# zju3dv/Diffuman4D

Measured on NVIDIA H100. Metric: unet_window_denoise_steps_per_sec, higher is better.
Workload: dtype bf16

## Files before the change

diffuman4d_b200/csrc/common.cuh:

```cuda
#pragma once
#include <cuda.h>
#include <cuda_bf16.h>
#include <cuda_runtime.h>
#include <stdint.h>
#include <string>

namespace d4d {

typedef __nv_bfloat16 bf16;

void set_error(const std::string& msg);
#define D4D_CUDA_OK(expr)                                                                        \
  do {                                                                                           \
    cudaError_t _e = (expr);                                                                     \
    if (_e != cudaSuccess) {                                                                     \
      d4d::set_error(std::string(#expr) + " failed: " + cudaGetErrorString(_e) + " @" + __FILE__ + \
                     ":" + std::to_string(__LINE__));                                            \
      return 2;                                                                                  \
    }                                                                                            \
  } while (0)
#define D4D_REQUIRE(cond, msg)                                                                   \
  do {                                                                                           \
    if (!(cond)) {                                                                               \
      d4d::set_error(std::string("invalid argument: ") + msg + " (" #cond ") @" + __FILE__ + ":" + \
                     std::to_string(__LINE__));                                                  \
      return 1;                                                                                  \
    }                                                                                            \
  } while (0)

int make_tmap_2d(CUtensorMap* out, const void* base, uint64_t rows, uint64_t cols, uint64_t ld,
                 uint32_t box_cols, uint32_t box_rows, int swizzle_bytes);
int make_tmap_nhwc_store(CUtensorMap* out, void* base, uint64_t n, uint64_t h, uint64_t w, uint64_t c, uint32_t box_w,
                         uint32_t box_h, uint32_t box_n);
int make_tmap_nhwc(CUtensorMap* out, const void* base, uint64_t n, uint64_t h, uint64_t w, uint64_t c,
                   uint32_t box_c, uint32_t box_w, uint32_t box_h, uint32_t box_n, int swizzle_bytes, int stride = 1);

#ifdef __CUDACC__
__device__ __forceinline__ uint32_t smem_u32(const void* p) {
  return static_cast<uint32_t>(__cvta_generic_to_shared(p));
}
__device__ __forceinline__ bool elect_one() {
  uint32_t pred = 0;
  asm volatile(
      "{\n\t.reg .b32 rx;\n\t.reg .pred px;\n\t"
      "elect.sync rx|px, 0xffffffff;\n\t"
      "selp.b32 %0, 1, 0, px;\n\t}\n"
      : "=r"(pred));
  return pred != 0;
// ... 28 lines not shown
#endif
__device__ __forceinline__ void mbar_wait(uint64_t* bar, uint32_t parity) {
  uint32_t spins = 0;
  while (!mbar_try_wait(bar, parity)) {
    if (++spins > D4D_SPIN_LIMIT) {
      printf("d4d: mbarrier timeout block=(%d,%d) thread=%d bar=%u parity=%u\n", blockIdx.x, blockIdx.y,
             threadIdx.x, smem_u32(bar), parity);
      __trap();
    }
  }
}

__device__ __forceinline__ void fence_proxy_async_smem() {
  asm volatile("fence.proxy.async.shared::cta;" ::: "memory");
}
__device__ __forceinline__ void pdl_wait() { asm volatile("griddepcontrol.wait;" ::: "memory"); }
__device__ __forceinline__ void pdl_launch_dependents() { asm volatile("griddepcontrol.launch_dependents;" ::: "memory"); }
template <int R> __device__ __forceinline__ void setmaxnreg_dec() { asm volatile("setmaxnreg.dec.sync.aligned.u32 %0;" ::"n"(R)); }
template <int R> __device__ __forceinline__ void setmaxnreg_inc() { asm volatile("setmaxnreg.inc.sync.aligned.u32 %0;" ::"n"(R)); }

__device__ __forceinline__ void tma_prefetch_desc(const CUtensorMap* t) {
  asm volatile("prefetch.tensormap [%0];" ::"l"(reinterpret_cast<uint64_t>(t)) : "memory");
}
__device__ __forceinline__ void tma_load_2d(void* dst, const CUtensorMap* t, uint64_t* bar, int c0, int c1) {
  asm volatile(
      "cp.async.bulk.tensor.2d.shared::cluster.global.tile.mbarrier::complete_tx::bytes [%0], [%1, {%3, %4}], [%2];"
      ::"r"(smem_u32(dst)), "l"(reinterpret_cast<uint64_t>(t)), "r"(smem_u32(bar)), "r"(c0), "r"(c1)
      : "memory");
}
__device__ __forceinline__ void tma_load_4d(void* dst, const CUtensorMap* t, uint64_t* bar, int c0, int c1, int c2,
                                            int c3) {
  asm volatile(
      "cp.async.bulk.tensor.4d.shared::cluster.global.tile.mbarrier::complete_tx::bytes [%0], [%1, {%3, %4, %5, %6}], [%2];"
      ::"r"(smem_u32(dst)), "l"(reinterpret_cast<uint64_t>(t)), "r"(smem_u32(bar)), "r"(c0), "r"(c1), "r"(c2),
      "r"(c3)
      : "memory");
}

__device__ __forceinline__ void tma_store_2d(const CUtensorMap* t, const void* src, int c0, int c1) {
  asm volatile("cp.async.bulk.tensor.2d.global.shared::cta.bulk_group [%0, {%2, %3}], [%1];"
               ::"l"(reinterpret_cast<uint64_t>(t)), "r"(smem_u32(src)), "r"(c0), "r"(c1) : "memory");
}
__device__ __forceinline__ void tma_store_4d(const CUtensorMap* t, const void* src, int c0, int c1, int c2, int c3) {
  asm volatile("cp.async.bulk.tensor.4d.global.shared::cta.bulk_group [%0, {%2, %3, %4, %5}], [%1];"
               ::"l"(reinterpret_cast<uint64_t>(t)), "r"(smem_u32(src)), "r"(c0), "r"(c1), "r"(c2), "r"(c3) : "memory");
}
__device__ __forceinline__ void bulk_commit_group() { asm volatile("cp.async.bulk.commit_group;" ::: "memory"); }
template <int N> __device__ __forceinline__ void bulk_wait_group_read() {
  asm volatile("cp.async.bulk.wait_group.read %0;" ::"n"(N) : "memory");
}
template <int N> __device__ __forceinline__ void bulk_wait_group() {
  asm volatile("cp.async.bulk.wait_group %0;" ::"n"(N) : "memory");
}

__device__ __forceinline__ uint32_t pack_bf16x2(float lo, float hi) {
  __nv_bfloat162 v = __floats2bfloat162_rn(lo, hi);
  return *reinterpret_cast<uint32_t*>(&v);
}
__device__ __forceinline__ float2 unpack_bf16x2(uint32_t u) {
  __nv_bfloat162 v = *reinterpret_cast<__nv_bfloat162*>(&u);
// ... 17 lines not shown
```

diffuman4d_b200/csrc/gemm_wgmma.cu:

```cuda
#include "kernels.h"
#include "wgmma.cuh"

namespace d4d {

namespace {

constexpr int BLOCK_M = 128;
constexpr int BLOCK_K = 64;
constexpr int A_BYTES = BLOCK_M * BLOCK_K * 2;
constexpr int BAR_BYTES = 1024;
constexpr int NUM_THREADS = 384;
constexpr int MAX_SMEM = 227 * 1024;

template <int BN>
struct GemmCfg {
  static constexpr int STAGE_BYTES = A_BYTES + BN * BLOCK_K * 2;
  static constexpr int STAGES_FIT = (MAX_SMEM - 1024 - BAR_BYTES) / STAGE_BYTES;
  static constexpr int STAGES = STAGES_FIT > 8 ? 8 : STAGES_FIT;
  static constexpr int SMEM = 1024 + BAR_BYTES + STAGES * STAGE_BYTES;
};

struct TileCoord {
  int m0;
  int n_img0, y0, x0;
  int pa, pb;
};

template <bool kConv>
__device__ __forceinline__ void tile_coords(const GemmKernelArgs& a, int m_tile, TileCoord& t) {
  if (!kConv) {
    t.m0 = m_tile * BLOCK_M;
    t.n_img0 = t.y0 = t.x0 = 0;
    t.pa = t.pb = 0;
  } else {
// ... 20 lines not shown
    valid = row < a.M;
    img = a.rows_per_image > 0 ? static_cast<int>(row / a.rows_per_image) : 0;
  } else {
    const int bx = rr % a.BW;
    const int r2 = rr / a.BW;
    const int by = r2 % a.BH;
    const int bn = r2 / a.BH;
    const int x = tc.x0 + bx, y = tc.y0 + by, n = tc.n_img0 + bn;
    valid = (x < a.W) && (y < a.H) && (n < a.n_img);
    row = (static_cast<long long>(n) * a.out_H + (y * a.out_sy + a.out_oy + tc.pa)) * a.out_W + (x * a.out_sx + a.out_ox + tc.pb);
    img = n;
  }
}

enum : int { E_BIAS = 1, E_ROWVEC = 2, E_ACT = 4, E_RES = 8, E_STATS = 16, E_KV = 32, E_ALL = 63 };

template <int BN, bool kGeglu, bool kConv, int kEpi>
__global__ void __launch_bounds__(NUM_THREADS, 1)
gemm_wgmma_kernel(const __grid_constant__ CUtensorMap tmap_a, const __grid_constant__ CUtensorMap tmap_a2,
                  const __grid_constant__ CUtensorMap tmap_b, const GemmKernelArgs a) {
  using Cfg = GemmCfg<BN>;
  constexpr int STAGES = Cfg::STAGES;
  extern __shared__ uint8_t smem_raw[];
  uint8_t* smem = reinterpret_cast<uint8_t*>((reinterpret_cast<uintptr_t>(smem_raw) + 1023) & ~uintptr_t(1023));
  uint64_t* full = reinterpret_cast<uint64_t*>(smem);
  uint64_t* empty = full + STAGES;
  uint8_t* ring = smem + BAR_BYTES;

  const int warp = __shfl_sync(0xffffffffu, threadIdx.x >> 5, 0);
  const int lane = threadIdx.x & 31;
  const int total_tiles = a.m_tiles * a.n_tiles;

  if (threadIdx.x == 0) {
    tma_prefetch_desc(&tmap_a);
    tma_prefetch_desc(&tmap_b);
    if (a.kb_split < a.k_blocks) tma_prefetch_desc(&tmap_a2);
    for (int i = 0; i < STAGES; ++i) {
      mbar_init(&full[i], 1);
      mbar_init(&empty[i], 2);
    }
    fence_mbar_init();
  }
  __syncthreads();
  pdl_wait();
  pdl_launch_dependents();

  if (warp < 4) {
    setmaxnreg_dec<40>();
    if (threadIdx.x == 0) {
      const uint32_t tx_bytes = A_BYTES + static_cast<uint32_t>(a.block_n) * BLOCK_K * 2;
      int stage = 0;
      uint32_t phase = 0;
      for (int tile = blockIdx.x; tile < total_tiles; tile += gridDim.x) {
        const int m_tile = tile / a.n_tiles;
        const int n_tile = tile % a.n_tiles;
// ... 18 lines not shown
          }
          if (++stage == STAGES) { stage = 0; phase ^= 1; }
        }
      }
    }
    return;
  }

  setmaxnreg_inc<232>();
  const int wg = (warp >> 2) - 1;
  const int wq = warp & 3;
  const bool wg_leader = (threadIdx.x & 127) == 0;
  const int r_base = wg * 64 + wq * 16 + (lane >> 2);
  const int c_base = 2 * (lane & 3);
  const uint32_t ring_u32 = smem_u32(ring);

  int stage = 0;
  uint32_t phase = 0;
  float acc[BN / 2];
  for (int tile = blockIdx.x; tile < total_tiles; tile += gridDim.x) {
    const int m_tile = tile / a.n_tiles;
    const int n_tile = tile % a.n_tiles;
    TileCoord tc;
    tile_coords<kConv>(a, m_tile, tc);
    const int n0 = n_tile * a.block_n;

    int prev_stage = -1;
    for (int kb = 0; kb < a.k_blocks; ++kb) {
      mbar_wait(&full[stage], phase);
      const uint32_t sa = ring_u32 + stage * Cfg::STAGE_BYTES + wg * 64 * 128;
      const uint32_t sb = ring_u32 + stage * Cfg::STAGE_BYTES + A_BYTES;
      const uint64_t adesc = make_wgmma_desc(sa, 16, 1024);
      const uint64_t bdesc = make_wgmma_desc(sb, 16, 1024);
      wgmma_fence();
#pragma unroll
      for (int k = 0; k < BLOCK_K / 16; ++k) {
        const int scale_d = (kb | k) != 0 ? 1 : 0;
        if constexpr (BN == 64) wgmma_ss_n64(acc, adesc + 2 * k, bdesc + 2 * k, scale_d);
        else if constexpr (BN == 128) wgmma_ss_n128(acc, adesc + 2 * k, bdesc + 2 * k, scale_d);
        else wgmma_ss_n256(acc, adesc + 2 * k, bdesc + 2 * k, scale_d);
      }
      wgmma_commit();
      wgmma_wait<1>();
      if (prev_stage >= 0 && wg_leader) mbar_arrive(&empty[prev_stage]);
      prev_stage = stage;
      if (++stage == STAGES) { stage = 0; phase ^= 1; }
    }
    wgmma_wait<0>();
    wgmma_fence_regs(acc);
    if (wg_leader) mbar_arrive(&empty[prev_stage]);

    long long rows[2];
    int imgs[2];
    bool valid[2];
    row_of<kConv>(a, tc, r_base, rows[0], imgs[0], valid[0]);
    row_of<kConv>(a, tc, r_base + 8, rows[1], imgs[1], valid[1]);

    if constexpr (kGeglu) {
      const bool has_bias = (kEpi & E_BIAS) && a.bias != nullptr;
#pragma unroll
      for (int p = 0; p < BN / 16; ++p) {
        if (16 * p >= a.block_n || n0 + 16 * p >= a.N) break;
        float2 ba = make_float2(0.f, 0.f), bg = make_float2(0.f, 0.f);
        if (has_bias) {
          ba = __ldg(reinterpret_cast<const float2*>(a.bias + n0 + 16 * p + c_base));
          bg = __ldg(reinterpret_cast<const float2*>(a.bias + n0 + 16 * p + 8 + c_base));
        }
        const int ocol = n0 / 2 + 8 * p + c_base;
#pragma unroll
        for (int h = 0; h < 2; ++h) {
          if (!valid[h]) continue;
          const float a0 = acc[8 * p + 2 * h] + ba.x, a1 = acc[8 * p + 2 * h + 1] + ba.y;
          const float g0 = acc[8 * p + 4 + 2 * h] + bg.x, g1 = acc[8 * p + 4 + 2 * h + 1] + bg.y;
          *reinterpret_cast<uint32_t*>(a.out + static_cast<size_t>(rows[h]) * a.ldo + ocol) =
              pack_bf16x2(a0 * gelu_erf_f(g0), a1 * gelu_erf_f(g1));
        }
      }
    } else {
      const bool has_bias = (kEpi & E_BIAS) && a.bias != nullptr, has_rv = (kEpi & E_ROWVEC) && a.rowvec != nullptr;
      const bool has_res = (kEpi & E_RES) && a.residual != nullptr, has_stats = (kEpi & E_STATS) && a.stats != nullptr;
      const bool has_act = (kEpi & E_ACT) && a.act == 1, has_scale = (kEpi & E_ACT) && a.out_scale != 1.0f;
      const bool has_kv = (kEpi & E_KV) && a.kv_world > 0;
      const long long row0 = __shfl_sync(0xffffffffu, rows[0], 0);
      const bool stats_on = has_stats && __shfl_sync(0xffffffffu, valid[0] ? 1 : 0, 0);
      const int stats_img = !kConv ? static_cast<int>(row0 / a.stats_rows) : __shfl_sync(0xffffffffu, imgs[0], 0);
#pragma unroll
      for (int j = 0; j < BN / 8; ++j) {
        const int cl = 8 * j + c_base;
        const int col = n0 + cl;
        if (8 * j >= a.block_n || n0 + 8 * j >= a.N) break;
        float2 b2 = make_float2(0.f, 0.f);
        if (has_bias) b2 = __ldg(reinterpret_cast<const float2*>(a.bias + col));
        float sv[2][2];
#pragma unroll
        for (int h = 0; h < 2; ++h) {
          sv[h][0] = sv[h][1] = 0.f;
          if (!valid[h]) continue;
          float f0 = acc[4 * j + 2 * h] + b2.x, f1 = acc[4 * j + 2 * h + 1] + b2.y;
          if (has_rv) {
            const float2 v = unpack_bf16x2(*reinterpret_cast<const uint32_t*>(a.rowvec + static_cast<size_t>(imgs[h]) * a.ld_rowvec + col));
            f0 += v.x; f1 += v.y;
          }
          if (has_act) { f0 = silu_f(f0); f1 = silu_f(f1); }
          if (has_scale) { f0 *= a.out_scale; f1 *= a.out_scale; }
          if (has_res) {
            const float2 v = unpack_bf16x2(*reinterpret_cast<const uint32_t*>(a.residual + static_cast<size_t>(rows[h]) * a.ld_res + col));
            f0 += v.x; f1 += v.y;
          }
          const uint32_t o = pack_bf16x2(f0, f1);
          if (has_stats) {
            const float2 rv = unpack_bf16x2(o);
            sv[h][0] = rv.x; sv[h][1] = rv.y;
          }
          if (has_kv && col >= a.kv_col0) {
            const long long half = rows[h] / a.kv_rows_local;
            const long long grow = half * a.kv_rows_global + a.kv_row_offset + (rows[h] - half * a.kv_rows_local);
            const size_t off = static_cast<size_t>(grow) * a.kv_ld + (col - a.kv_col0);
#pragma unroll 1
            for (int rk = 0; rk < a.kv_world; ++rk) *reinterpret_cast<uint32_t*>(a.kv_dst[rk] + off) = o;
          } else {
            *reinterpret_cast<uint32_t*>(a.out + static_cast<size_t>(rows[h]) * a.ldo + col) = o;
          }
        }
        if (has_stats) {
          float s0 = sv[0][0] + sv[1][0], s1 = sv[0][1] + sv[1][1];
          float q0 = sv[0][0] * sv[0][0] + sv[1][0] * sv[1][0], q1 = sv[0][1] * sv[0][1] + sv[1][1] * sv[1][1];
#pragma unroll
          for (int m = 4; m < 32; m <<= 1) {
            s0 += __shfl_xor_sync(0xffffffffu, s0, m);
            s1 += __shfl_xor_sync(0xffffffffu, s1, m);
            q0 += __shfl_xor_sync(0xffffffffu, q0, m);
            q1 += __shfl_xor_sync(0xffffffffu, q1, m);
          }
          if (stats_on && lane < 4) {
            unsigned long long* st = reinterpret_cast<unsigned long long*>(a.stats) + (static_cast<size_t>(stats_img) * a.N + col) * 2;
            atomicAdd(st + 0, static_cast<unsigned long long>(__float2ll_rn(s0 * kGnSumScale)));
            atomicAdd(st + 1, static_cast<unsigned long long>(__float2ll_rn(q0 * kGnSqScale)));
            atomicAdd(st + 2, static_cast<unsigned long long>(__float2ll_rn(s1 * kGnSumScale)));
            atomicAdd(st + 3, static_cast<unsigned long long>(__float2ll_rn(q1 * kGnSqScale)));
          }
        }
      }
    }
  }
}

}

int gemm_prepare(const GemmDesc& d, GemmLaunch* L) {
  D4D_REQUIRE(d.N % 16 == 0, "GEMM N must be a multiple of 16");
  D4D_REQUIRE(d.out != nullptr && d.A != nullptr && d.Wt != nullptr, "null operand");
  GemmKernelArgs& a = L->args;
  memset(&a, 0, sizeof(a));
  int dev = 0, sms = 0;
  D4D_CUDA_OK(cudaGetDevice(&dev));
  D4D_CUDA_OK(cudaDeviceGetAttribute(&sms, cudaDevAttrMultiProcessorCount, dev));
  int bn = d.block_n;
  if (bn <= 0) {
    const long long rows = d.conv ? static_cast<long long>(d.n_img) * d.H * d.W : d.M;
    const long long m_tiles_est = (rows + BLOCK_M - 1) / BLOCK_M;
    long long best_cost = -1;
    for (int c = 64; c <= 256; c *= 2) {
      const long long tiles = m_tiles_est * ((d.N + c - 1) / c);
      const long long waves = (tiles + sms - 1) / sms;
      const long long cost = waves * (c + 64) + (static_cast<long long>((d.N + c - 1) / c) * c - d.N) / 4;
      if (best_cost < 0 || cost <= best_cost) { best_cost = cost; bn = c; }
    }
  }
  D4D_REQUIRE(bn >= 16 && bn <= 256 && bn % 16 == 0 && (d.block_n <= 0 || d.N % bn == 0), "no valid block_n");
  a.block_n = bn;
  a.n_tiles = (d.N + bn - 1) / bn;
  a.N = d.N;
  a.bias = d.bias;
  a.rowvec = d.rowvec;
  a.ld_rowvec = d.ld_rowvec;
  a.rows_per_image = d.rows_per_image;
  a.residual = d.residual;
// ... 24 lines not shown
    D4D_REQUIRE(d.A2 == nullptr || d.K1 % BLOCK_K == 0, "two-source GEMM needs K1 % 64 == 0");
    a.mode = 0;
    a.M = d.M;
    a.m_tiles = (d.M + BLOCK_M - 1) / BLOCK_M;
    a.kb_split = (d.K1 + BLOCK_K - 1) / BLOCK_K;
    const int kb2 = d.A2 ? (d.K2 + BLOCK_K - 1) / BLOCK_K : 0;
    a.k_blocks = a.kb_split + kb2;
    const int K = d.K1 + (d.A2 ? d.K2 : 0);
    if (int rc = make_tmap_2d(&L->tmap_a, d.A, d.M, d.K1, d.lda, BLOCK_K, BLOCK_M, 128)) return rc;
    if (d.A2) {
      if (int rc = make_tmap_2d(&L->tmap_a2, d.A2, d.M, d.K2, d.lda2, BLOCK_K, BLOCK_M, 128)) return rc;
    } else {
      L->tmap_a2 = L->tmap_a;
    }
    if (int rc = make_tmap_2d(&L->tmap_b, d.Wt, d.N, K, K, BLOCK_K, bn, 128)) return rc;
  } else {
    D4D_REQUIRE(d.Cin % 8 == 0, "conv Cin must be a multiple of 8");
    D4D_REQUIRE(d.conv_kind >= 0 && d.conv_kind <= 3, "conv_kind");
    D4D_REQUIRE(d.conv_kind != 1 || (d.H % 2 == 0 && d.W % 2 == 0), "stride-2 conv needs even H, W");
    a.mode = 1;
    a.n_img = d.n_img; a.Cin = d.Cin;
    a.in_stride = 1; a.out_sy = a.out_sx = 1; a.out_oy = a.out_ox = 0;
    a.n_phases = 1;
    if (d.conv_kind >= 2) {
      const int pa = d.conv_kind == 3 ? 0 : d.up_a, pb = d.conv_kind == 3 ? 0 : d.up_b;
      a.n_taps = 4;
      for (int t = 0; t < 4; ++t) {
        a.tap_dy[t] = static_cast<signed char>((t >> 1) + pa - 1);
        a.tap_dx[t] = static_cast<signed char>((t & 1) + pb - 1);
      }
// ... 15 lines not shown
    a.k_blocks = a.n_taps * a.cin_blocks;
    a.kb_split = a.k_blocks;
    int bw = 16; while (bw > a.W) bw >>= 1;
    int bh = 128 / bw; while (bh > a.H && bh > 1) bh >>= 1;
    int bnimg = 128 / (bw * bh);
    D4D_REQUIRE(bw * bh * bnimg == 128 && bnimg <= 256, "conv tile shape");
    D4D_REQUIRE(d.stats == nullptr || (bw * bh) % 32 == 0, "statistics need 32-row warps inside one image");
    a.BW = bw; a.BH = bh; a.BN = bnimg;
    a.tiles_x = (a.W + bw - 1) / bw;
    a.tiles_y = (a.H + bh - 1) / bh;
    const int tiles_n = (d.n_img + bnimg - 1) / bnimg;
    a.tiles_per_phase = a.tiles_x * a.tiles_y * tiles_n;
    a.m_tiles = a.tiles_per_phase * a.n_phases;
    a.M *= a.n_phases;
    if (int rc = make_tmap_nhwc(&L->tmap_a, d.A, d.n_img, d.H, d.W, d.Cin, BLOCK_K, bw, bh, bnimg, 128, a.in_stride)) return rc;
    L->tmap_a2 = L->tmap_a;
    const uint64_t kw = static_cast<uint64_t>(a.n_taps) * d.Cin;
    if (int rc = make_tmap_2d(&L->tmap_b, d.Wt, static_cast<uint64_t>(d.N) * a.n_phases, kw, kw, BLOCK_K, bn, 128)) return rc;
  }
  const int total = a.m_tiles * a.n_tiles;
  L->grid = total < sms ? total : sms;
  return 0;
}

namespace {

using GemmKernelFn = void (*)(const CUtensorMap, const CUtensorMap, const CUtensorMap, const GemmKernelArgs);
struct GemmVariant {
  int bn;
  bool geglu, conv;
  int epi;
  GemmKernelFn fn;
  int smem;
};
#define D4D_GV(BN, G, C, E) {BN, G, C, E, gemm_wgmma_kernel<BN, G, C, E>, GemmCfg<BN>::SMEM}
#define D4D_GV_SET(BN)                                                                                                \
                                         \
  D4D_GV(BN, false, false, 0), D4D_GV(BN, false, false, E_BIAS), D4D_GV(BN, false, false, E_BIAS | E_RES),           \
  D4D_GV(BN, false, false, E_BIAS | E_RES | E_STATS), D4D_GV(BN, false, false, E_ALL),                                \
                                                            \
  D4D_GV(BN, false, true, E_BIAS | E_ROWVEC | E_STATS), D4D_GV(BN, false, true, E_BIAS | E_RES | E_STATS),           \
  D4D_GV(BN, false, true, E_BIAS | E_STATS), D4D_GV(BN, false, true, E_ALL),                                          \
                                                                    \
  D4D_GV(BN, true, false, E_BIAS)
const GemmVariant kGemmVariants[] = {
    D4D_GV_SET(128), D4D_GV_SET(256),
    D4D_GV(64, false, false, E_ALL), D4D_GV(64, false, true, E_ALL), D4D_GV(64, true, false, E_BIAS),
};
#undef D4D_GV_SET
#undef D4D_GV
constexpr int kNumGemmVariants = sizeof(kGemmVariants) / sizeof(kGemmVariants[0]);

int gemm_variant_of(const GemmKernelArgs& a) {
  const bool conv = a.mode != 0, geglu = a.geglu != 0;
  const int bn = a.block_n <= 64 ? 64 : a.block_n <= 128 ? 128 : 256;
  int need = 0;
  if (a.bias) need |= E_BIAS;
  if (!geglu) {
    if (a.rowvec) need |= E_ROWVEC;
    if (a.act == 1 || a.out_scale != 1.0f) need |= E_ACT;
    if (a.residual) need |= E_RES;
    if (a.stats) need |= E_STATS;
    if (a.kv_world > 0) need |= E_KV;
  }
  int generic = -1;
  for (int i = 0; i < kNumGemmVariants; ++i) {
    const GemmVariant& v = kGemmVariants[i];
    if (v.bn != bn || v.geglu != geglu || v.conv != conv) continue;
    if (v.epi == need) return i;
    if ((v.epi & need) == need && (generic < 0 || v.epi == E_ALL)) generic = i;
  }
  return generic;
}

}

int gemm_run(const GemmLaunch& L, cudaStream_t stream) {
  static PerDeviceOnce attr_once[kNumGemmVariants];
  const int vi = gemm_variant_of(L.args);
  D4D_REQUIRE(vi >= 0, "no GEMM kernel instantiation covers this launch");
  const GemmVariant& v = kGemmVariants[vi];
  if (int rc = ensure_dyn_smem(v.fn, v.smem, attr_once[vi])) return rc;
  D4D_CUDA_OK(launch_pdl(v.fn, dim3(L.grid), dim3(NUM_THREADS), v.smem, stream, L.tmap_a, L.tmap_a2, L.tmap_b, L.args));
  D4D_CUDA_OK(cudaGetLastError());
  return 0;
}

double gemm_flops(const GemmLaunch& L) {
  return 2.0 * static_cast<double>(L.args.M) * L.args.N * (static_cast<double>(L.args.k_blocks) * BLOCK_K);
}

}
```

diffuman4d_b200/csrc/kernels.h:

```cpp
#pragma once
#include <cstdlib>
#include <mutex>
#include <utility>
#include <string.h>

#include "common.cuh"

namespace d4d {

constexpr float kGnSumScale = 268435456.f;
constexpr float kGnSqScale = 16777216.f;

struct GemmKernelArgs {
  int M, N, k_blocks, block_n, n_tiles, m_tiles;
  int mode;
  int kb_split;
  int H, W, n_img, Cin, cin_blocks, BW, BH, BN, tiles_x, tiles_y;
  int n_taps, in_stride, out_sy, out_sx, out_oy, out_ox, out_H, out_W;
  int n_phases, tiles_per_phase;
  signed char tap_dy[9], tap_dx[9];
  const float* bias;
  const bf16* rowvec;
  int ld_rowvec, rows_per_image;
  const bf16* residual;
  int ld_res;
  bf16* out;
  int ldo;
  int geglu;
  int act;
  float out_scale;
  long long* stats;
  int stats_rows;
  int kv_world, kv_col0, kv_ld;
  long long kv_rows_local, kv_rows_global, kv_row_offset;
  bf16* kv_dst[8];
};

struct GemmDesc {
  const bf16* A = nullptr;
  int lda = 0, K1 = 0;
  const bf16* A2 = nullptr;
  int lda2 = 0, K2 = 0;
// ... 8 lines not shown
  int ldo = 0;
  int geglu = 0;
  int act = 0;
  float out_scale = 1.0f;
  int block_n = 0;
  long long* stats = nullptr;
  int stats_rows = 0;
  int kv_world = 0, kv_col0 = 0, kv_ld = 0;
  long long kv_rows_local = 0, kv_rows_global = 0, kv_row_offset = 0;
  bf16* kv_dst[8] = {nullptr, nullptr, nullptr, nullptr, nullptr, nullptr, nullptr, nullptr};
  int conv = 0, n_img = 0, H = 0, W = 0, Cin = 0;
  int conv_kind = 0, up_a = 0, up_b = 0;
};

struct GemmLaunch {
  CUtensorMap tmap_a, tmap_a2, tmap_b;
  GemmKernelArgs args;
  int grid;
};

int gemm_prepare(const GemmDesc& d, GemmLaunch* L);
int gemm_run(const GemmLaunch& L, cudaStream_t stream);
double gemm_flops(const GemmLaunch& L);

struct AttnDesc {
  const bf16* q = nullptr;
  const bf16* k = nullptr;
  const bf16* v = nullptr;
  int ld_qkv = 0;
  bf16* out = nullptr;
  int ld_out = 0;
// ... 108 lines not shown
```

diffuman4d_b200/csrc/tmap.cu:

```cuda
#include "common.cuh"

#include <mutex>

namespace d4d {

typedef CUresult (*EncodeTiledFn)(CUtensorMap*, CUtensorMapDataType, cuuint32_t, void*, const cuuint64_t*,
                                  const cuuint64_t*, const cuuint32_t*, const cuuint32_t*, CUtensorMapInterleave,
                                  CUtensorMapSwizzle, CUtensorMapL2promotion, CUtensorMapFloatOOBfill);

static EncodeTiledFn get_encode_fn() {
  static EncodeTiledFn fn = nullptr;
  static std::once_flag once;
  std::call_once(once, [] {
    void* p = nullptr;
    cudaDriverEntryPointQueryResult q;
    cudaError_t e = cudaGetDriverEntryPoint("cuTensorMapEncodeTiled", &p, cudaEnableDefault, &q);
    if (e == cudaSuccess && q == cudaDriverEntryPointSuccess) fn = reinterpret_cast<EncodeTiledFn>(p);
    else (void)cudaGetLastError();
  });
  return fn;
}

static CUtensorMapSwizzle swz(int bytes) {
  switch (bytes) {
// ... 43 lines not shown
  cuuint64_t gstr[3] = {c * 2, w * c * 2, h * w * c * 2};
  D4D_REQUIRE(stride >= 1 && stride <= 8 && box_w * stride <= 256 && box_h * stride <= 256, "TMA traversal stride");
  const cuuint32_t s = static_cast<cuuint32_t>(stride);
  cuuint32_t box[4] = {box_c, box_w * s, box_h * s, box_n};
  cuuint32_t estr[4] = {1, s, s, 1};
  CUresult r = fn(out, CU_TENSOR_MAP_DATA_TYPE_BFLOAT16, 4, const_cast<void*>(base), gdim, gstr, box, estr,
                  CU_TENSOR_MAP_INTERLEAVE_NONE, swz(swizzle_bytes), CU_TENSOR_MAP_L2_PROMOTION_L2_256B,
                  CU_TENSOR_MAP_FLOAT_OOB_FILL_NONE);
  if (r != CUDA_SUCCESS) {
    set_error("cuTensorMapEncodeTiled(4d) failed, CUresult=" + std::to_string(static_cast<int>(r)));
    return 2;
  }
  return 0;
}

int make_tmap_nhwc_store(CUtensorMap* out, void* base, uint64_t n, uint64_t h, uint64_t w, uint64_t c, uint32_t box_w,
                         uint32_t box_h, uint32_t box_n) {
  return make_tmap_nhwc(out, base, n, h, w, c, 32, box_w, box_h, box_n, 64, 1);
}

}
```

diffuman4d_b200/csrc/wgmma.cuh:

```cuda
#pragma once
#include <stdint.h>

namespace d4d {

__device__ __forceinline__ void wgmma_fence() { asm volatile("wgmma.fence.sync.aligned;" ::: "memory"); }
__device__ __forceinline__ void wgmma_commit() { asm volatile("wgmma.commit_group.sync.aligned;" ::: "memory"); }
template <int N> __device__ __forceinline__ void wgmma_wait() {
  asm volatile("wgmma.wait_group.sync.aligned %0;" ::"n"(N) : "memory");
}
template <int R> __device__ __forceinline__ void wgmma_fence_regs(float (&d)[R]) {
#pragma unroll
  for (int i = 0; i < R; ++i) asm volatile("" : "+f"(d[i])::"memory");
}

__device__ __forceinline__ uint64_t make_wgmma_desc(uint32_t saddr, uint32_t lbo_bytes, uint32_t sbo_bytes) {
  uint64_t d = 0;
  d |= static_cast<uint64_t>((saddr >> 4) & 0x3FFFu);
  d |= static_cast<uint64_t>((lbo_bytes >> 4) & 0x3FFFu) << 16;
  d |= static_cast<uint64_t>((sbo_bytes >> 4) & 0x3FFFu) << 32;
  d |= 1ull << 62;
  return d;
}


// ... 3 lines not shown
      "setp.ne.b32 p, %34, 0;\n\t"
      "wgmma.mma_async.sync.aligned.m64n64k16.f32.bf16.bf16 {%0, %1, %2, %3, %4, %5, %6, %7, %8, %9, %10, %11, %12, %13, %14, %15, %16, %17, %18, %19, %20, %21, %22, %23, %24, %25, %26, %27, %28, %29, %30, %31}, %32, %33, p, 1, 1, 0, 0;\n\t}\n"
      : "+f"(d[0]), "+f"(d[1]), "+f"(d[2]), "+f"(d[3]), "+f"(d[4]), "+f"(d[5]), "+f"(d[6]), "+f"(d[7]), "+f"(d[8]), "+f"(d[9]), "+f"(d[10]), "+f"(d[11]), "+f"(d[12]), "+f"(d[13]), "+f"(d[14]), "+f"(d[15]), "+f"(d[16]), "+f"(d[17]), "+f"(d[18]), "+f"(d[19]), "+f"(d[20]), "+f"(d[21]), "+f"(d[22]), "+f"(d[23]), "+f"(d[24]), "+f"(d[25]), "+f"(d[26]), "+f"(d[27]), "+f"(d[28]), "+f"(d[29]), "+f"(d[30]), "+f"(d[31])
      : "l"(a_desc), "l"(b_desc), "r"(scale_d));
}

__device__ __forceinline__ void wgmma_ss_n128(float (&d)[64], uint64_t a_desc, uint64_t b_desc, int scale_d) {
  asm volatile(
      "{\n\t.reg .pred p;\n\t"
      "setp.ne.b32 p, %66, 0;\n\t"
      "wgmma.mma_async.sync.aligned.m64n128k16.f32.bf16.bf16 {%0, %1, %2, %3, %4, %5, %6, %7, %8, %9, %10, %11, %12, %13, %14, %15, %16, %17, %18, %19, %20, %21, %22, %23, %24, %25, %26, %27, %28, %29, %30, %31, %32, %33, %34, %35, %36, %37, %38, %39, %40, %41, %42, %43, %44, %45, %46, %47, %48, %49, %50, %51, %52, %53, %54, %55, %56, %57, %58, %59, %60, %61, %62, %63}, %64, %65, p, 1, 1, 0, 0;\n\t}\n"
      : "+f"(d[0]), "+f"(d[1]), "+f"(d[2]), "+f"(d[3]), "+f"(d[4]), "+f"(d[5]), "+f"(d[6]), "+f"(d[7]), "+f"(d[8]), "+f"(d[9]), "+f"(d[10]), "+f"(d[11]), "+f"(d[12]), "+f"(d[13]), "+f"(d[14]), "+f"(d[15]), "+f"(d[16]), "+f"(d[17]), "+f"(d[18]), "+f"(d[19]), "+f"(d[20]), "+f"(d[21]), "+f"(d[22]), "+f"(d[23]), "+f"(d[24]), "+f"(d[25]), "+f"(d[26]), "+f"(d[27]), "+f"(d[28]), "+f"(d[29]), "+f"(d[30]), "+f"(d[31]), "+f"(d[32]), "+f"(d[33]), "+f"(d[34]), "+f"(d[35]), "+f"(d[36]), "+f"(d[37]), "+f"(d[38]), "+f"(d[39]), "+f"(d[40]), "+f"(d[41]), "+f"(d[42]), "+f"(d[43]), "+f"(d[44]), "+f"(d[45]), "+f"(d[46]), "+f"(d[47]), "+f"(d[48]), "+f"(d[49]), "+f"(d[50]), "+f"(d[51]), "+f"(d[52]), "+f"(d[53]), "+f"(d[54]), "+f"(d[55]), "+f"(d[56]), "+f"(d[57]), "+f"(d[58]), "+f"(d[59]), "+f"(d[60]), "+f"(d[61]), "+f"(d[62]), "+f"(d[63])
      : "l"(a_desc), "l"(b_desc), "r"(scale_d));
}

__device__ __forceinline__ void wgmma_ss_n256(float (&d)[128], uint64_t a_desc, uint64_t b_desc, int scale_d) {
  asm volatile(
      "{\n\t.reg .pred p;\n\t"
      "setp.ne.b32 p, %130, 0;\n\t"
      "wgmma.mma_async.sync.aligned.m64n256k16.f32.bf16.bf16 {%0, %1, %2, %3, %4, %5, %6, %7, %8, %9, %10, %11, %12, %13, %14, %15, %16, %17, %18, %19, %20, %21, %22, %23, %24, %25, %26, %27, %28, %29, %30, %31, %32, %33, %34, %35, %36, %37, %38, %39, %40, %41, %42, %43, %44, %45, %46, %47, %48, %49, %50, %51, %52, %53, %54, %55, %56, %57, %58, %59, %60, %61, %62, %63, %64, %65, %66, %67, %68, %69, %70, %71, %72, %73, %74, %75, %76, %77, %78, %79, %80, %81, %82, %83, %84, %85, %86, %87, %88, %89, %90, %91, %92, %93, %94, %95, %96, %97, %98, %99, %100, %101, %102, %103, %104, %105, %106, %107, %108, %109, %110, %111, %112, %113, %114, %115, %116, %117, %118, %119, %120, %121, %122, %123, %124, %125, %126, %127}, %128, %129, p, 1, 1, 0, 0;\n\t}\n"
      : "+f"(d[0]), "+f"(d[1]), "+f"(d[2]), "+f"(d[3]), "+f"(d[4]), "+f"(d[5]), "+f"(d[6]), "+f"(d[7]), "+f"(d[8]), "+f"(d[9]), "+f"(d[10]), "+f"(d[11]), "+f"(d[12]), "+f"(d[13]), "+f"(d[14]), "+f"(d[15]), "+f"(d[16]), "+f"(d[17]), "+f"(d[18]), "+f"(d[19]), "+f"(d[20]), "+f"(d[21]), "+f"(d[22]), "+f"(d[23]), "+f"(d[24]), "+f"(d[25]), "+f"(d[26]), "+f"(d[27]), "+f"(d[28]), "+f"(d[29]), "+f"(d[30]), "+f"(d[31]), "+f"(d[32]), "+f"(d[33]), "+f"(d[34]), "+f"(d[35]), "+f"(d[36]), "+f"(d[37]), "+f"(d[38]), "+f"(d[39]), "+f"(d[40]), "+f"(d[41]), "+f"(d[42]), "+f"(d[43]), "+f"(d[44]), "+f"(d[45]), "+f"(d[46]), "+f"(d[47]), "+f"(d[48]), "+f"(d[49]), "+f"(d[50]), "+f"(d[51]), "+f"(d[52]), "+f"(d[53]), "+f"(d[54]), "+f"(d[55]), "+f"(d[56]), "+f"(d[57]), "+f"(d[58]), "+f"(d[59]), "+f"(d[60]), "+f"(d[61]), "+f"(d[62]), "+f"(d[63]), "+f"(d[64]), "+f"(d[65]), "+f"(d[66]), "+f"(d[67]), "+f"(d[68]), "+f"(d[69]), "+f"(d[70]), "+f"(d[71]), "+f"(d[72]), "+f"(d[73]), "+f"(d[74]), "+f"(d[75]), "+f"(d[76]), "+f"(d[77]), "+f"(d[78]), "+f"(d[79]), "+f"(d[80]), "+f"(d[81]), "+f"(d[82]), "+f"(d[83]), "+f"(d[84]), "+f"(d[85]), "+f"(d[86]), "+f"(d[87]), "+f"(d[88]), "+f"(d[89]), "+f"(d[90]), "+f"(d[91]), "+f"(d[92]), "+f"(d[93]), "+f"(d[94]), "+f"(d[95]), "+f"(d[96]), "+f"(d[97]), "+f"(d[98]), "+f"(d[99]), "+f"(d[100]), "+f"(d[101]), "+f"(d[102]), "+f"(d[103]), "+f"(d[104]), "+f"(d[105]), "+f"(d[106]), "+f"(d[107]), "+f"(d[108]), "+f"(d[109]), "+f"(d[110]), "+f"(d[111]), "+f"(d[112]), "+f"(d[113]), "+f"(d[114]), "+f"(d[115]), "+f"(d[116]), "+f"(d[117]), "+f"(d[118]), "+f"(d[119]), "+f"(d[120]), "+f"(d[121]), "+f"(d[122]), "+f"(d[123]), "+f"(d[124]), "+f"(d[125]), "+f"(d[126]), "+f"(d[127])
      : "l"(a_desc), "l"(b_desc), "r"(scale_d));
}

__device__ __forceinline__ void wgmma_rs_n64_bmn(float (&d)[32], const uint32_t (&a)[4], uint64_t b_desc) {
  asm volatile(
      "wgmma.mma_async.sync.aligned.m64n64k16.f32.bf16.bf16 {%0, %1, %2, %3, %4, %5, %6, %7, %8, %9, %10, %11, %12, %13, %14, %15, %16, %17, %18, %19, %20, %21, %22, %23, %24, %25, %26, %27, %28, %29, %30, %31}, {%32, %33, %34, %35}, %36, 1, 1, 1, 1;\n"
      : "+f"(d[0]), "+f"(d[1]), "+f"(d[2]), "+f"(d[3]), "+f"(d[4]), "+f"(d[5]), "+f"(d[6]), "+f"(d[7]), "+f"(d[8]), "+f"(d[9]), "+f"(d[10]), "+f"(d[11]), "+f"(d[12]), "+f"(d[13]), "+f"(d[14]), "+f"(d[15]), "+f"(d[16]), "+f"(d[17]), "+f"(d[18]), "+f"(d[19]), "+f"(d[20]), "+f"(d[21]), "+f"(d[22]), "+f"(d[23]), "+f"(d[24]), "+f"(d[25]), "+f"(d[26]), "+f"(d[27]), "+f"(d[28]), "+f"(d[29]), "+f"(d[30]), "+f"(d[31])
      : "r"(a[0]), "r"(a[1]), "r"(a[2]), "r"(a[3]), "l"(b_desc));
}
// ... 3 lines not shown
```

Measured before the change: 9.310.

## Stage GEMM epilogue through swizzled smem with TMA stores and residual prefetch

```diff
diff --git a/diffuman4d_b200/csrc/common.cuh b/diffuman4d_b200/csrc/common.cuh
--- a/diffuman4d_b200/csrc/common.cuh
+++ b/diffuman4d_b200/csrc/common.cuh
@@ -30,8 +30,6 @@
 
 int make_tmap_2d(CUtensorMap* out, const void* base, uint64_t rows, uint64_t cols, uint64_t ld,
                  uint32_t box_cols, uint32_t box_rows, int swizzle_bytes);
-int make_tmap_nhwc_store(CUtensorMap* out, void* base, uint64_t n, uint64_t h, uint64_t w, uint64_t c, uint32_t box_w,
-                         uint32_t box_h, uint32_t box_n);
 int make_tmap_nhwc(CUtensorMap* out, const void* base, uint64_t n, uint64_t h, uint64_t w, uint64_t c,
                    uint32_t box_c, uint32_t box_w, uint32_t box_h, uint32_t box_n, int swizzle_bytes, int stride = 1);
 
@@ -90,6 +88,17 @@
 __device__ __forceinline__ void fence_proxy_async_smem() {
   asm volatile("fence.proxy.async.shared::cta;" ::: "memory");
 }
+__device__ __forceinline__ void named_barrier_sync(int id, int threads) {
+  asm volatile("bar.sync %0, %1;" ::"r"(id), "r"(threads) : "memory");
+}
+__device__ __forceinline__ void st_shared_u32(uint32_t addr, uint32_t v) {
+  asm volatile("st.shared.b32 [%0], %1;" ::"r"(addr), "r"(v) : "memory");
+}
+__device__ __forceinline__ uint32_t ld_shared_u32(uint32_t addr) {
+  uint32_t v;
+  asm volatile("ld.shared.b32 %0, [%1];" : "=r"(v) : "r"(addr) : "memory");
+  return v;
+}
 __device__ __forceinline__ void pdl_wait() { asm volatile("griddepcontrol.wait;" ::: "memory"); }
 __device__ __forceinline__ void pdl_launch_dependents() { asm volatile("griddepcontrol.launch_dependents;" ::: "memory"); }
 template <int R> __device__ __forceinline__ void setmaxnreg_dec() { asm volatile("setmaxnreg.dec.sync.aligned.u32 %0;" ::"n"(R)); }
@@ -116,10 +125,6 @@
 __device__ __forceinline__ void tma_store_2d(const CUtensorMap* t, const void* src, int c0, int c1) {
   asm volatile("cp.async.bulk.tensor.2d.global.shared::cta.bulk_group [%0, {%2, %3}], [%1];"
                ::"l"(reinterpret_cast<uint64_t>(t)), "r"(smem_u32(src)), "r"(c0), "r"(c1) : "memory");
-}
-__device__ __forceinline__ void tma_store_4d(const CUtensorMap* t, const void* src, int c0, int c1, int c2, int c3) {
-  asm volatile("cp.async.bulk.tensor.4d.global.shared::cta.bulk_group [%0, {%2, %3, %4, %5}], [%1];"
-               ::"l"(reinterpret_cast<uint64_t>(t)), "r"(smem_u32(src)), "r"(c0), "r"(c1), "r"(c2), "r"(c3) : "memory");
 }
 __device__ __forceinline__ void bulk_commit_group() { asm volatile("cp.async.bulk.commit_group;" ::: "memory"); }
 template <int N> __device__ __forceinline__ void bulk_wait_group_read() {
diff --git a/diffuman4d_b200/csrc/gemm_wgmma.cu b/diffuman4d_b200/csrc/gemm_wgmma.cu
--- a/diffuman4d_b200/csrc/gemm_wgmma.cu
+++ b/diffuman4d_b200/csrc/gemm_wgmma.cu
@@ -12,12 +12,16 @@
 constexpr int NUM_THREADS = 384;
 constexpr int MAX_SMEM = 227 * 1024;
 
-template <int BN>
+constexpr int SLAB_COLS = 32;
+constexpr int SLAB_BYTES = 64 * SLAB_COLS * 2;
+
+template <int BN, bool kStaged>
 struct GemmCfg {
   static constexpr int STAGE_BYTES = A_BYTES + BN * BLOCK_K * 2;
-  static constexpr int STAGES_FIT = (MAX_SMEM - 1024 - BAR_BYTES) / STAGE_BYTES;
+  static constexpr int STAGING_BYTES = kStaged ? 2 * 64 * BN * 2 : 0;
+  static constexpr int STAGES_FIT = (MAX_SMEM - 1024 - BAR_BYTES - STAGING_BYTES) / STAGE_BYTES;
   static constexpr int STAGES = STAGES_FIT > 8 ? 8 : STAGES_FIT;
-  static constexpr int SMEM = 1024 + BAR_BYTES + STAGES * STAGE_BYTES;
+  static constexpr int SMEM = 1024 + BAR_BYTES + STAGES * STAGE_BYTES + STAGING_BYTES;
 };
 
 struct TileCoord {
@@ -68,17 +72,21 @@
 }
 
 enum : int { E_BIAS = 1, E_ROWVEC = 2, E_ACT = 4, E_RES = 8, E_STATS = 16, E_KV = 32, E_ALL = 63 };
+__host__ __device__ constexpr bool gemm_staged(bool conv, int epi) { return !conv && !(epi & E_KV); }
 
 template <int BN, bool kGeglu, bool kConv, int kEpi>
 __global__ void __launch_bounds__(NUM_THREADS, 1)
 gemm_wgmma_kernel(const __grid_constant__ CUtensorMap tmap_a, const __grid_constant__ CUtensorMap tmap_a2,
-                  const __grid_constant__ CUtensorMap tmap_b, const GemmKernelArgs a) {
-  using Cfg = GemmCfg<BN>;
+                  const __grid_constant__ CUtensorMap tmap_b, const __grid_constant__ CUtensorMap tmap_c,
+                  const __grid_constant__ CUtensorMap tmap_r, const GemmKernelArgs a) {
+  constexpr bool kStaged = gemm_staged(kConv, kEpi);
+  using Cfg = GemmCfg<BN, kStaged>;
   constexpr int STAGES = Cfg::STAGES;
   extern __shared__ uint8_t smem_raw[];
   uint8_t* smem = reinterpret_cast<uint8_t*>((reinterpret_cast<uintptr_t>(smem_raw) + 1023) & ~uintptr_t(1023));
   uint64_t* full = reinterpret_cast<uint64_t*>(smem);
   uint64_t* empty = full + STAGES;
+  uint64_t* res_full = empty + STAGES;
   uint8_t* ring = smem + BAR_BYTES;
 
   const int warp = __shfl_sync(0xffffffffu, threadIdx.x >> 5, 0);
@@ -93,6 +101,8 @@
       mbar_init(&full[i], 1);
       mbar_init(&empty[i], 2);
     }
+    mbar_init(&res_full[0], 1);
+    mbar_init(&res_full[1], 1);
     fence_mbar_init();
   }
   __syncthreads();
@@ -141,6 +151,13 @@
   const int r_base = wg * 64 + wq * 16 + (lane >> 2);
   const int c_base = 2 * (lane & 3);
   const uint32_t ring_u32 = smem_u32(ring);
+  const bool staged = kStaged && a.staged;
+  uint8_t* stg = ring + STAGES * Cfg::STAGE_BYTES + wg * 64 * BN * 2;
+  const uint32_t stg_u32 = smem_u32(stg) + (r_base - wg * 64) * 64 + c_base * 2;
+  const int stg_xor = (lane >> 3) & 3;
+  const bool has_res = (kEpi & E_RES) && !kGeglu && a.residual != nullptr;
+  const int out_cols = kGeglu ? a.N / 2 : a.N;
+  uint32_t res_phase = 0;
 
   int stage = 0;
   uint32_t phase = 0;
@@ -151,6 +168,11 @@
     TileCoord tc;
     tile_coords<kConv>(a, m_tile, tc);
     const int n0 = n_tile * a.block_n;
+    const int ocol0 = kGeglu ? n0 / 2 : n0;
+    const int ocols = min(kGeglu ? a.block_n / 2 : a.block_n, out_cols - ocol0);
+    const int n_slabs = (ocols + SLAB_COLS - 1) / SLAB_COLS;
+    const int orow0 = tc.m0 + wg * 64;
+    const bool stg_live = staged && orow0 < a.M;
 
     int prev_stage = -1;
     for (int kb = 0; kb < a.k_blocks; ++kb) {
@@ -165,9 +187,19 @@
         const int scale_d = (kb | k) != 0 ? 1 : 0;
         if constexpr (BN == 64) wgmma_ss_n64(acc, adesc + 2 * k, bdesc + 2 * k, scale_d);
         else if constexpr (BN == 128) wgmma_ss_n128(acc, adesc + 2 * k, bdesc + 2 * k, scale_d);
+        else if constexpr (BN == 160) wgmma_ss_n160(acc, adesc + 2 * k, bdesc + 2 * k, scale_d);
+        else if constexpr (BN == 192) wgmma_ss_n192(acc, adesc + 2 * k, bdesc + 2 * k, scale_d);
         else wgmma_ss_n256(acc, adesc + 2 * k, bdesc + 2 * k, scale_d);
       }
       wgmma_commit();
+      if (kb == 0 && staged && wg_leader) {
+        bulk_wait_group_read<0>();
+        if (has_res && stg_live) {
+          mbar_expect_tx(&res_full[wg], n_slabs * SLAB_BYTES);
+          for (int s = 0; s < n_slabs; ++s)
+            tma_load_2d(stg + s * SLAB_BYTES, &tmap_r, &res_full[wg], ocol0 + s * SLAB_COLS, orow0);
+        }
+      }
       wgmma_wait<1>();
       if (prev_stage >= 0 && wg_leader) mbar_arrive(&empty[prev_stage]);
       prev_stage = stage;
@@ -182,6 +214,16 @@
     bool valid[2];
     row_of<kConv>(a, tc, r_base, rows[0], imgs[0], valid[0]);
     row_of<kConv>(a, tc, r_base + 8, rows[1], imgs[1], valid[1]);
+    if (staged) {
+      named_barrier_sync(1 + wg, 128);
+      if (has_res && stg_live) {
+        mbar_wait(&res_full[wg], res_phase);
+        res_phase ^= 1;
+      }
+    }
+    auto stg_addr = [&](int j, int h) {
+      return stg_u32 + h * 8 * 64 + (j >> 2) * SLAB_BYTES + (((j & 3) ^ stg_xor) << 4);
+    };
 
     if constexpr (kGeglu) {
       const bool has_bias = (kEpi & E_BIAS) && a.bias != nullptr;
@@ -199,13 +241,14 @@
           if (!valid[h]) continue;
           const float a0 = acc[8 * p + 2 * h] + ba.x, a1 = acc[8 * p + 2 * h + 1] + ba.y;
           const float g0 = acc[8 * p + 4 + 2 * h] + bg.x, g1 = acc[8 * p + 4 + 2 * h + 1] + bg.y;
-          *reinterpret_cast<uint32_t*>(a.out + static_cast<size_t>(rows[h]) * a.ldo + ocol) =
-              pack_bf16x2(a0 * gelu_erf_f(g0), a1 * gelu_erf_f(g1));
+          const uint32_t o = pack_bf16x2(a0 * gelu_erf_f(g0), a1 * gelu_erf_f(g1));
+          if (staged) st_shared_u32(stg_addr(p, h), o);
+          else *reinterpret_cast<uint32_t*>(a.out + static_cast<size_t>(rows[h]) * a.ldo + ocol) = o;
         }
       }
     } else {
       const bool has_bias = (kEpi & E_BIAS) && a.bias != nullptr, has_rv = (kEpi & E_ROWVEC) && a.rowvec != nullptr;
-      const bool has_res = (kEpi & E_RES) && a.residual != nullptr, has_stats = (kEpi & E_STATS) && a.stats != nullptr;
+      const bool has_stats = (kEpi & E_STATS) && a.stats != nullptr;
       const bool has_act = (kEpi & E_ACT) && a.act == 1, has_scale = (kEpi & E_ACT) && a.out_scale != 1.0f;
       const bool has_kv = (kEpi & E_KV) && a.kv_world > 0;
       const long long row0 = __shfl_sync(0xffffffffu, rows[0], 0);
@@ -231,7 +274,8 @@
           if (has_act) { f0 = silu_f(f0); f1 = silu_f(f1); }
           if (has_scale) { f0 *= a.out_scale; f1 *= a.out_scale; }
           if (has_res) {
-            const float2 v = unpack_bf16x2(*reinterpret_cast<const uint32_t*>(a.residual + static_cast<size_t>(rows[h]) * a.ld_res + col));
+            const float2 v = unpack_bf16x2(staged ? ld_shared_u32(stg_addr(j, h))
+                                                  : *reinterpret_cast<const uint32_t*>(a.residual + static_cast<size_t>(rows[h]) * a.ld_res + col));
             f0 += v.x; f1 += v.y;
           }
           const uint32_t o = pack_bf16x2(f0, f1);
@@ -245,6 +289,8 @@
             const size_t off = static_cast<size_t>(grow) * a.kv_ld + (col - a.kv_col0);
 #pragma unroll 1
             for (int rk = 0; rk < a.kv_world; ++rk) *reinterpret_cast<uint32_t*>(a.kv_dst[rk] + off) = o;
+          } else if (staged) {
+            st_shared_u32(stg_addr(j, h), o);
           } else {
             *reinterpret_cast<uint32_t*>(a.out + static_cast<size_t>(rows[h]) * a.ldo + col) = o;
           }
@@ -269,7 +315,16 @@
         }
       }
     }
-  }
+    if (staged) {
+      fence_proxy_async_smem();
+      named_barrier_sync(1 + wg, 128);
+      if (wg_leader && stg_live) {
+        for (int s = 0; s < n_slabs; ++s) tma_store_2d(&tmap_c, stg + s * SLAB_BYTES, ocol0 + s * SLAB_COLS, orow0);
+        bulk_commit_group();
+      }
+    }
+  }
+  if (staged && wg_leader) bulk_wait_group<0>();
 }
 
 }
@@ -287,7 +342,8 @@
     const long long rows = d.conv ? static_cast<long long>(d.n_img) * d.H * d.W : d.M;
     const long long m_tiles_est = (rows + BLOCK_M - 1) / BLOCK_M;
     long long best_cost = -1;
-    for (int c = 64; c <= 256; c *= 2) {
+    for (int c : {64, 128, 160, 192, 256}) {
+      if (d.geglu && c % 64 != 0) continue;
       const long long tiles = m_tiles_est * ((d.N + c - 1) / c);
       const long long waves = (tiles + sms - 1) / sms;
       const long long cost = waves * (c + 64) + (static_cast<long long>((d.N + c - 1) / c) * c - d.N) / 4;
@@ -342,6 +398,15 @@
       L->tmap_a2 = L->tmap_a;
     }
     if (int rc = make_tmap_2d(&L->tmap_b, d.Wt, d.N, K, K, BLOCK_K, bn, 128)) return rc;
+    const auto aligned16 = [](const void* p) { return (reinterpret_cast<uintptr_t>(p) & 15) == 0; };
+    a.staged = d.kv_world == 0 && (d.geglu ? bn % (2 * SLAB_COLS) : bn % SLAB_COLS) == 0 && aligned16(d.out) &&
+               (d.residual == nullptr || aligned16(d.residual));
+    L->tmap_c = L->tmap_r = L->tmap_a;
+    if (a.staged) {
+      if (int rc = make_tmap_2d(&L->tmap_c, d.out, d.M, d.geglu ? d.N / 2 : d.N, d.ldo, SLAB_COLS, 64, 64)) return rc;
+      if (d.residual && !d.geglu)
+        if (int rc = make_tmap_2d(&L->tmap_r, d.residual, d.M, d.N, d.ld_res, SLAB_COLS, 64, 64)) return rc;
+    }
   } else {
     D4D_REQUIRE(d.Cin % 8 == 0, "conv Cin must be a multiple of 8");
     D4D_REQUIRE(d.conv_kind >= 0 && d.conv_kind <= 3, "conv_kind");
@@ -387,7 +452,7 @@
     a.m_tiles = a.tiles_per_phase * a.n_phases;
     a.M *= a.n_phases;
     if (int rc = make_tmap_nhwc(&L->tmap_a, d.A, d.n_img, d.H, d.W, d.Cin, BLOCK_K, bw, bh, bnimg, 128, a.in_stride)) return rc;
-    L->tmap_a2 = L->tmap_a;
+    L->tmap_a2 = L->tmap_c = L->tmap_r = L->tmap_a;
     const uint64_t kw = static_cast<uint64_t>(a.n_taps) * d.Cin;
     if (int rc = make_tmap_2d(&L->tmap_b, d.Wt, static_cast<uint64_t>(d.N) * a.n_phases, kw, kw, BLOCK_K, bn, 128)) return rc;
   }
@@ -398,7 +463,8 @@
 
 namespace {
 
-using GemmKernelFn = void (*)(const CUtensorMap, const CUtensorMap, const CUtensorMap, const GemmKernelArgs);
+using GemmKernelFn = void (*)(const CUtensorMap, const CUtensorMap, const CUtensorMap, const CUtensorMap,
+                              const CUtensorMap, const GemmKernelArgs);
 struct GemmVariant {
   int bn;
   bool geglu, conv;
@@ -406,27 +472,29 @@
   GemmKernelFn fn;
   int smem;
 };
-#define D4D_GV(BN, G, C, E) {BN, G, C, E, gemm_wgmma_kernel<BN, G, C, E>, GemmCfg<BN>::SMEM}
-#define D4D_GV_SET(BN)                                                                                                \
+#define D4D_GV(BN, G, C, E) {BN, G, C, E, gemm_wgmma_kernel<BN, G, C, E>, GemmCfg<BN, gemm_staged(C, E)>::SMEM}
+#define D4D_GV_PLAIN(BN)                                                                                              \
                                          \
   D4D_GV(BN, false, false, 0), D4D_GV(BN, false, false, E_BIAS), D4D_GV(BN, false, false, E_BIAS | E_RES),           \
-  D4D_GV(BN, false, false, E_BIAS | E_RES | E_STATS), D4D_GV(BN, false, false, E_ALL),                                \
+  D4D_GV(BN, false, false, E_BIAS | E_RES | E_STATS), D4D_GV(BN, false, false, E_ALL)
+#define D4D_GV_CONV(BN)                                                                                               \
                                                             \
   D4D_GV(BN, false, true, E_BIAS | E_ROWVEC | E_STATS), D4D_GV(BN, false, true, E_BIAS | E_RES | E_STATS),           \
-  D4D_GV(BN, false, true, E_BIAS | E_STATS), D4D_GV(BN, false, true, E_ALL),                                          \
-                                                                    \
-  D4D_GV(BN, true, false, E_BIAS)
+  D4D_GV(BN, false, true, E_BIAS | E_STATS), D4D_GV(BN, false, true, E_ALL)
 const GemmVariant kGemmVariants[] = {
-    D4D_GV_SET(128), D4D_GV_SET(256),
+    D4D_GV_PLAIN(128), D4D_GV_CONV(128), D4D_GV(128, true, false, E_BIAS),
+    D4D_GV_PLAIN(160), D4D_GV_CONV(160),
+    D4D_GV_PLAIN(192),
+    D4D_GV_PLAIN(256), D4D_GV_CONV(256), D4D_GV(256, true, false, E_BIAS),
     D4D_GV(64, false, false, E_ALL), D4D_GV(64, false, true, E_ALL), D4D_GV(64, true, false, E_BIAS),
 };
-#undef D4D_GV_SET
+#undef D4D_GV_CONV
+#undef D4D_GV_PLAIN
 #undef D4D_GV
 constexpr int kNumGemmVariants = sizeof(kGemmVariants) / sizeof(kGemmVariants[0]);
 
-int gemm_variant_of(const GemmKernelArgs& a) {
+int gemm_variant_at(const GemmKernelArgs& a, int bn) {
   const bool conv = a.mode != 0, geglu = a.geglu != 0;
-  const int bn = a.block_n <= 64 ? 64 : a.block_n <= 128 ? 128 : 256;
   int need = 0;
   if (a.bias) need |= E_BIAS;
   if (!geglu) {
@@ -446,6 +514,15 @@
   return generic;
 }
 
+int gemm_variant_of(const GemmKernelArgs& a) {
+  for (int bn : {64, 128, 160, 192, 256}) {
+    if (bn < a.block_n) continue;
+    const int vi = gemm_variant_at(a, bn);
+    if (vi >= 0) return vi;
+  }
+  return -1;
+}
+
 }
 
 int gemm_run(const GemmLaunch& L, cudaStream_t stream) {
@@ -454,7 +531,8 @@
   D4D_REQUIRE(vi >= 0, "no GEMM kernel instantiation covers this launch");
   const GemmVariant& v = kGemmVariants[vi];
   if (int rc = ensure_dyn_smem(v.fn, v.smem, attr_once[vi])) return rc;
-  D4D_CUDA_OK(launch_pdl(v.fn, dim3(L.grid), dim3(NUM_THREADS), v.smem, stream, L.tmap_a, L.tmap_a2, L.tmap_b, L.args));
+  D4D_CUDA_OK(launch_pdl(v.fn, dim3(L.grid), dim3(NUM_THREADS), v.smem, stream, L.tmap_a, L.tmap_a2, L.tmap_b, L.tmap_c, L.tmap_r,
+                         L.args));
   D4D_CUDA_OK(cudaGetLastError());
   return 0;
 }
diff --git a/diffuman4d_b200/csrc/kernels.h b/diffuman4d_b200/csrc/kernels.h
--- a/diffuman4d_b200/csrc/kernels.h
+++ b/diffuman4d_b200/csrc/kernels.h
@@ -26,6 +26,7 @@
   int ld_res;
   bf16* out;
   int ldo;
+  int staged;
   int geglu;
   int act;
   float out_scale;
@@ -64,7 +65,7 @@
 };
 
 struct GemmLaunch {
-  CUtensorMap tmap_a, tmap_a2, tmap_b;
+  CUtensorMap tmap_a, tmap_a2, tmap_b, tmap_c, tmap_r;
   GemmKernelArgs args;
   int grid;
 };
diff --git a/diffuman4d_b200/csrc/tmap.cu b/diffuman4d_b200/csrc/tmap.cu
--- a/diffuman4d_b200/csrc/tmap.cu
+++ b/diffuman4d_b200/csrc/tmap.cu
@@ -81,9 +81,4 @@
   return 0;
 }
 
-int make_tmap_nhwc_store(CUtensorMap* out, void* base, uint64_t n, uint64_t h, uint64_t w, uint64_t c, uint32_t box_w,
-                         uint32_t box_h, uint32_t box_n) {
-  return make_tmap_nhwc(out, base, n, h, w, c, 32, box_w, box_h, box_n, 64, 1);
 }
-
-}
diff --git a/diffuman4d_b200/csrc/wgmma.cuh b/diffuman4d_b200/csrc/wgmma.cuh
--- a/diffuman4d_b200/csrc/wgmma.cuh
+++ b/diffuman4d_b200/csrc/wgmma.cuh
@@ -41,6 +41,24 @@
       : "l"(a_desc), "l"(b_desc), "r"(scale_d));
 }
 
+__device__ __forceinline__ void wgmma_ss_n160(float (&d)[80], uint64_t a_desc, uint64_t b_desc, int scale_d) {
+  asm volatile(
+      "{\n\t.reg .pred p;\n\t"
+      "setp.ne.b32 p, %82, 0;\n\t"
+      "wgmma.mma_async.sync.aligned.m64n160k16.f32.bf16.bf16 {%0, %1, %2, %3, %4, %5, %6, %7, %8, %9, %10, %11, %12, %13, %14, %15, %16, %17, %18, %19, %20, %21, %22, %23, %24, %25, %26, %27, %28, %29, %30, %31, %32, %33, %34, %35, %36, %37, %38, %39, %40, %41, %42, %43, %44, %45, %46, %47, %48, %49, %50, %51, %52, %53, %54, %55, %56, %57, %58, %59, %60, %61, %62, %63, %64, %65, %66, %67, %68, %69, %70, %71, %72, %73, %74, %75, %76, %77, %78, %79}, %80, %81, p, 1, 1, 0, 0;\n\t}\n"
+      : "+f"(d[0]), "+f"(d[1]), "+f"(d[2]), "+f"(d[3]), "+f"(d[4]), "+f"(d[5]), "+f"(d[6]), "+f"(d[7]), "+f"(d[8]), "+f"(d[9]), "+f"(d[10]), "+f"(d[11]), "+f"(d[12]), "+f"(d[13]), "+f"(d[14]), "+f"(d[15]), "+f"(d[16]), "+f"(d[17]), "+f"(d[18]), "+f"(d[19]), "+f"(d[20]), "+f"(d[21]), "+f"(d[22]), "+f"(d[23]), "+f"(d[24]), "+f"(d[25]), "+f"(d[26]), "+f"(d[27]), "+f"(d[28]), "+f"(d[29]), "+f"(d[30]), "+f"(d[31]), "+f"(d[32]), "+f"(d[33]), "+f"(d[34]), "+f"(d[35]), "+f"(d[36]), "+f"(d[37]), "+f"(d[38]), "+f"(d[39]), "+f"(d[40]), "+f"(d[41]), "+f"(d[42]), "+f"(d[43]), "+f"(d[44]), "+f"(d[45]), "+f"(d[46]), "+f"(d[47]), "+f"(d[48]), "+f"(d[49]), "+f"(d[50]), "+f"(d[51]), "+f"(d[52]), "+f"(d[53]), "+f"(d[54]), "+f"(d[55]), "+f"(d[56]), "+f"(d[57]), "+f"(d[58]), "+f"(d[59]), "+f"(d[60]), "+f"(d[61]), "+f"(d[62]), "+f"(d[63]), "+f"(d[64]), "+f"(d[65]), "+f"(d[66]), "+f"(d[67]), "+f"(d[68]), "+f"(d[69]), "+f"(d[70]), "+f"(d[71]), "+f"(d[72]), "+f"(d[73]), "+f"(d[74]), "+f"(d[75]), "+f"(d[76]), "+f"(d[77]), "+f"(d[78]), "+f"(d[79])
+      : "l"(a_desc), "l"(b_desc), "r"(scale_d));
+}
+
+__device__ __forceinline__ void wgmma_ss_n192(float (&d)[96], uint64_t a_desc, uint64_t b_desc, int scale_d) {
+  asm volatile(
+      "{\n\t.reg .pred p;\n\t"
+      "setp.ne.b32 p, %98, 0;\n\t"
+      "wgmma.mma_async.sync.aligned.m64n192k16.f32.bf16.bf16 {%0, %1, %2, %3, %4, %5, %6, %7, %8, %9, %10, %11, %12, %13, %14, %15, %16, %17, %18, %19, %20, %21, %22, %23, %24, %25, %26, %27, %28, %29, %30, %31, %32, %33, %34, %35, %36, %37, %38, %39, %40, %41, %42, %43, %44, %45, %46, %47, %48, %49, %50, %51, %52, %53, %54, %55, %56, %57, %58, %59, %60, %61, %62, %63, %64, %65, %66, %67, %68, %69, %70, %71, %72, %73, %74, %75, %76, %77, %78, %79, %80, %81, %82, %83, %84, %85, %86, %87, %88, %89, %90, %91, %92, %93, %94, %95}, %96, %97, p, 1, 1, 0, 0;\n\t}\n"
+      : "+f"(d[0]), "+f"(d[1]), "+f"(d[2]), "+f"(d[3]), "+f"(d[4]), "+f"(d[5]), "+f"(d[6]), "+f"(d[7]), "+f"(d[8]), "+f"(d[9]), "+f"(d[10]), "+f"(d[11]), "+f"(d[12]), "+f"(d[13]), "+f"(d[14]), "+f"(d[15]), "+f"(d[16]), "+f"(d[17]), "+f"(d[18]), "+f"(d[19]), "+f"(d[20]), "+f"(d[21]), "+f"(d[22]), "+f"(d[23]), "+f"(d[24]), "+f"(d[25]), "+f"(d[26]), "+f"(d[27]), "+f"(d[28]), "+f"(d[29]), "+f"(d[30]), "+f"(d[31]), "+f"(d[32]), "+f"(d[33]), "+f"(d[34]), "+f"(d[35]), "+f"(d[36]), "+f"(d[37]), "+f"(d[38]), "+f"(d[39]), "+f"(d[40]), "+f"(d[41]), "+f"(d[42]), "+f"(d[43]), "+f"(d[44]), "+f"(d[45]), "+f"(d[46]), "+f"(d[47]), "+f"(d[48]), "+f"(d[49]), "+f"(d[50]), "+f"(d[51]), "+f"(d[52]), "+f"(d[53]), "+f"(d[54]), "+f"(d[55]), "+f"(d[56]), "+f"(d[57]), "+f"(d[58]), "+f"(d[59]), "+f"(d[60]), "+f"(d[61]), "+f"(d[62]), "+f"(d[63]), "+f"(d[64]), "+f"(d[65]), "+f"(d[66]), "+f"(d[67]), "+f"(d[68]), "+f"(d[69]), "+f"(d[70]), "+f"(d[71]), "+f"(d[72]), "+f"(d[73]), "+f"(d[74]), "+f"(d[75]), "+f"(d[76]), "+f"(d[77]), "+f"(d[78]), "+f"(d[79]), "+f"(d[80]), "+f"(d[81]), "+f"(d[82]), "+f"(d[83]), "+f"(d[84]), "+f"(d[85]), "+f"(d[86]), "+f"(d[87]), "+f"(d[88]), "+f"(d[89]), "+f"(d[90]), "+f"(d[91]), "+f"(d[92]), "+f"(d[93]), "+f"(d[94]), "+f"(d[95])
+      : "l"(a_desc), "l"(b_desc), "r"(scale_d));
+}
+
 __device__ __forceinline__ void wgmma_ss_n256(float (&d)[128], uint64_t a_desc, uint64_t b_desc, int scale_d) {
   asm volatile(
       "{\n\t.reg .pred p;\n\t"
```

Result: faster. 10.46 (median of 6 runs) (+12.4%).
